# LepistaBioinformatics/blutils

Hardware: NVIDIA B200
Metric: consensus_queries_per_s (higher is better)
Workload: dtype u8

## Files before the change

### blutils_b200/csrc/blu_kernels.cu

```cuda
#include <cuda_runtime.h>

#include <climits>
#include <cstdio>

#include "blu_kernels.h"

namespace blu {

namespace {

constexpr int kRowCap = kWin / 26 + 16;
constexpr int kLongThreads = 512;
constexpr int kLongWarps = kLongThreads / 32;

__device__ __forceinline__ uint32_t smem_u32(const void* p) { return (uint32_t)__cvta_generic_to_shared(p); }
__device__ __forceinline__ uint32_t atoms_add(void* addr, uint32_t v) {
    uint32_t old;
    asm volatile("atom.shared.add.u32 %0, [%1], %2;" : "=r"(old) : "r"(smem_u32(addr)), "r"(v) : "memory");
    return old;
}

__device__ __forceinline__ void mbar_init(unsigned long long* bar, uint32_t count) {
    asm volatile("mbarrier.init.shared::cta.b64 [%0], %1;" ::"r"(smem_u32(bar)), "r"(count) : "memory");
    asm volatile("fence.mbarrier_init.release.cluster;" ::: "memory");
// ... 1377 lines not shown
    bool single;
    if (diverge > 0) {
        identity = __longlong_as_double((long long)S.bcast64[0]), idx = diverge - 1, level = diverge, single = false;
    } else {
        identity = ref.pident, idx = m - 1, level = m - 1, single = true;
    }
    for (int i = tid; i < n2; i += kLongThreads) {
        Q.bord[i] = i < g ? (uint16_t)i : (uint16_t)0xFFFFu;
        if (i < g) Q.key[i] = T.bean_key[T.lin_off[rows[Q.order[i]].lin] + level];
    }
    __syncthreads();
    block_bitonic_u16(Q.bord, n2, [&](int a, int b) { return Q.key[a] != Q.key[b] ? Q.key[a] < Q.key[b] : a < b; });
    for (int i = tid; i < g; i += kLongThreads) {
        const bool head = i == 0 || Q.key[Q.bord[i]] != Q.key[Q.bord[i - 1]];
        const bool kept = head || !acc_equal(rows[Q.order[Q.bord[i]]], rows[Q.order[Q.bord[i - 1]]], p.text);
        Q.tmp[i] = (uint16_t)((head ? 1 : 0) | (kept ? 2 : 0));
    }
    __syncthreads();
    const int nb = block_excl_scan_u16(Q.hb, g, [&](int i) { return (int)(Q.tmp[i] & 1u); }, S.scan_tot);
    const int nkept = block_excl_scan_u16(Q.kp, g, [&](int i) { return (int)((Q.tmp[i] >> 1) & 1u); }, S.scan_tot);
    for (int i = tid; i < g; i += kLongThreads) {
        const bool head = (Q.tmp[i] & 1u) != 0;
        if (head) Q.st[Q.hb[i]] = (uint16_t)i;
    }
    if (tid == 0) Q.st[nb] = (uint16_t)g;
    __syncthreads();
    for (int i = tid; i < g; i += kLongThreads) Q.hb[i] = (uint16_t)(Q.hb[i] + (Q.tmp[i] & 1u));
    int nb2 = 2;
    while (nb2 < nb) nb2 <<= 1;
    for (int j = tid; j < nb2; j += kLongThreads) Q.bsort[j] = j < nb ? (uint16_t)j : (uint16_t)0xFFFFu;
    __syncthreads();
    block_bitonic_u16(Q.bsort, nb2, [&](int a, int b) {
        const int oa = (int)Q.st[a + 1] - (int)Q.st[a], ob = (int)Q.st[b + 1] - (int)Q.st[b];
        if (oa != ob) return oa > ob;
        const uint32_t pa = T.lin_off[rows[Q.order[Q.bord[Q.st[a]]]].lin] + (uint32_t)level, pb = T.lin_off[rows[Q.order[Q.bord[Q.st[b]]]].lin] + (uint32_t)level;
        const uint32_t ia = T.ident_rank[pa], ib = T.ident_rank[pb];
        if (ia != ib) return ia < ib;
        return Q.key[Q.bord[Q.st[a]]] < Q.key[Q.bord[Q.st[b]]];
    });
    block_excl_scan_u16(Q.tmp, nb, [&](int j) { const int bb = Q.bsort[j]; return (int)Q.kp[Q.st[bb + 1]] - (int)Q.kp[Q.st[bb]]; }, S.scan_tot);
    for (int j = tid; j < nb; j += kLongThreads) Q.abeg[Q.bsort[j]] = Q.tmp[j];
    if (tid == 0) {
        const unsigned long long ri = atomicAdd(&p.ctr->rec_count, 1ull);
        const unsigned long long bb = atomicAdd(&p.ctr->bean_used, (unsigned long long)nb);
        const unsigned long long ab = atomicAdd(&p.ctr->acc_used, (unsigned long long)nkept);
        S.bcast64[1] = ri, S.bcast64[2] = bb, S.bcast64[3] = ab;
        if (ri >= p.rec_cap || bb + (unsigned long long)nb > p.bean_cap || ab + (unsigned long long)nkept > p.acc_cap) {
            p.ctr->cap_overflow = 1;
            S.bcast64[1] = ~0ull;
        }
    }
    __syncthreads();
    if (S.bcast64[1] == ~0ull) return DE_NONE;
    const unsigned long long ri = S.bcast64[1], bean_base = S.bcast64[2], acc_base = S.bcast64[3];
    for (int j = tid; j < nb; j += kLongThreads) {
        const int bb = Q.bsort[j];
        blu_bean bn;
        bn.first_lineage = rows[Q.order[Q.bord[Q.st[bb]]]].lin;
        bn.occurrences = (uint32_t)((int)Q.st[bb + 1] - (int)Q.st[bb]);
        bn.acc_begin = Q.abeg[bb];
        bn.n_acc = (uint32_t)((int)Q.kp[Q.st[bb + 1]] - (int)Q.kp[Q.st[bb]]);
        p.beans[bean_base + j] = bn;
    }
    for (int i = tid; i < g; i += kLongThreads)
        if (Q.kp[i + 1] != Q.kp[i]) {
            const int bb = (int)Q.hb[i] - 1;
            const TopRow& x = rows[Q.order[Q.bord[i]]];
            p.accs[acc_base + Q.abeg[bb] + (Q.kp[i] - Q.kp[Q.st[bb]])].ref = (x.acc_off << 16) | (unsigned long long)x.acc_len;
        }
    if (tid == 0) {
        blu_record* rec = p.records + ri;
        rec->query_off = s;
        rec->query_len = qlen;
        rec->n_rows = (uint32_t)nrows;
        rec->bit_score = mx;
        rec->perc_identity = ref.pident;
        rec->ref_lineage = ref.lin;
        rec->bean_base = (uint32_t)bean_base;
        rec->n_beans = (uint32_t)nb;
        rec->acc_base = (uint32_t)acc_base;
        rec->status = 1;
        rec->single_match = 0;
        rec->bean_level = (int8_t)level;
        rec->pad[0] = rec->pad[1] = 0;
        apply_cutoffs(T, ref.lin, identity, single && nb == 1, idx, rec);
    }
    return DE_NONE;
}

__global__ void __launch_bounds__(kLongThreads, 1) longrun_kernel(const __grid_constant__ RunParams p) {
    if (p.ctr->n_defer == 0) return;
    extern __shared__ __align__(128) uint8_t smem_raw[];
    LongSmem& S = *reinterpret_cast<LongSmem*>(smem_raw);
    const int tid = threadIdx.x, warp = tid >> 5, lane = tid & 31;
    const unsigned long long p_begin = p.begin == kBeginFromCounters ? p.ctr->next_begin : p.begin;
    if (tid == 0) mbar_init(&S.mbar, 1);
    __syncthreads();
    uint32_t phase = 0;
    const unsigned n_defer = p.ctr->n_defer < p.defer_cap ? p.ctr->n_defer : p.defer_cap;
    TopRow* const rows = p.big_rows + (size_t)blockIdx.x * kLongTopCap;
    unsigned long long* const cand = p.big_cand + (size_t)blockIdx.x * kLongTopCap;

    while (true) {
        __syncthreads();
        if (tid == 0) S.bcast[0] = (int)atomicAdd(&p.ctr->work_ticket, 1u);
        __syncthreads();
        const unsigned wi = (unsigned)S.bcast[0];
        if (wi >= n_defer) break;
        const unsigned long long entry = p.defer[wi];
        const unsigned long long s = entry >> 1;
        if (entry & 1) {
            if (tid == 0) {
                int head = 1;
                if (s > p_begin) {
                    long long q = (long long)s - 1;
                    while (q >= (long long)p_begin && p.text[q] == '\n') q--;
                    if (q >= (long long)p_begin) {
                        long long st = q;
                        while (st > (long long)p_begin && p.text[st - 1] != '\n') st--;
                        head = 0;
                        for (unsigned long long i = 0;; i++) {
                            if (s + i >= p.end || (unsigned long long)st + i > (unsigned long long)q) {
                                head = 1;
                                break;
                            }
                            uint8_t a = p.text[st + i], b = p.text[s + i];
                            if (a != b) {
                                head = 1;
                                break;
                            }
                            if (a == '\t') break;
                        }
                    }
                }
                S.bcast[1] = head;
            }
            __syncthreads();
            if (!S.bcast[1]) continue;
        }
        if (tid == 0) {
            int qn = 0;
            while (qn < kQidCache && s + qn < p.end) {
                const uint8_t b = p.text[s + qn];
                S.qid[qn++] = b;
                if (b == '\t') break;
            }
            S.bcast[4] = (qn > 0 && S.qid[qn - 1] == '\t') ? qn : 0;
        }
        __syncthreads();
        const int qn = S.bcast[4];
        long long mx = LLONG_MIN;
        long long cnt = 0, nrows = 0;
        unsigned long long cur = s;
        bool ended = false, hit_end = false, fail = false;
        while (true) {
            LongScan sc = long_scan(S, p, s, cur, phase, qn);
            if (sc.giant && sc.d == 0 && sc.ncomplete == 0) {
                if (!sc.at_end || p.final_chunk) {
                    if (tid == 0) report(p.ctr, DE_CARRY_TOO_BIG, cur);
                    fail = true;
                }
                hit_end = true;
                break;
            }
            const unsigned long long lo = cur & ~15ull;
            long long lm = LLONG_MIN;
            for (int i = tid; i < sc.d; i += kLongThreads) {
                const long long b = S.scan.bits[i];
                lm = b > lm ? b : lm;
            }
#pragma unroll
            for (int dd = 16; dd > 0; dd >>= 1) {
                const long long om = __shfl_xor_sync(0xffffffffu, lm, dd);
                lm = om > lm ? om : lm;
            }
            if (lane == 0) S.red_max[warp] = lm;
            __syncthreads();
            long long wm = LLONG_MIN;
            for (int i = 0; i < kLongWarps; i++) wm = S.red_max[i] > wm ? S.red_max[i] : wm;
            if (sc.d > 0 && wm > mx) {
                mx = wm;
                cnt = 0;
            }
            for (int b0 = 0; b0 < sc.d; b0 += kLongThreads) {
                const int i = b0 + tid;
                const bool top = i < sc.d && S.scan.bits[i] == mx;
                const unsigned bal = __ballot_sync(0xffffffffu, top);
                if (lane == 0) S.red_cnt[warp] = __popc(bal);
                __syncthreads();
                long long before = cnt;
                int total = 0;
                for (int k = 0; k < kLongWarps; k++) {
                    if (k < warp) before += S.red_cnt[k];
                    total += S.red_cnt[k];
                }
                if (top) {
                    const long long pos = before + __popc(bal & ((1u << lane) - 1u));
                    if (pos < kLongTopCap)
                        cand[pos] = ((lo + S.scan.W.row_s[i]) << 16) |
                                    (unsigned long long)(uint32_t)((int)S.scan.W.row_e[i + sc.eskip] - (int)S.scan.W.row_s[i]);
                }
                cnt += total;
                __syncthreads();
            }
            nrows += sc.d;
            if (sc.d < sc.ncomplete) {
                ended = true;
                break;
            }
            if (sc.at_end) {
                hit_end = true;
                break;
            }
            cur = sc.next;
        }
        if (fail) continue;
        if (!ended && hit_end && !p.final_chunk) {
            if (tid == 0) atomicMin(&p.ctr->tail_start, s);
            continue;
        }
        if (nrows == 0) continue;
        if (cnt > kLongTopCap) {
            if (tid == 0) report(p.ctr, DE_TOPGROUP_TOO_BIG, s);
            continue;
        }
        const int gcount = (int)cnt;
        uint32_t my_err = 0;
        unsigned long long my_off = 0;
        for (int i = tid; i < gcount; i += kLongThreads) {
            const unsigned long long off = cand[i] >> 16;
            const uint32_t err = heavy_parse_row(p.text + off, (int)(cand[i] & 0xFFFFull), off, p.T, rows[i]);
            if (err && !my_err) my_err = err, my_off = off;
        }
        if (my_err) report_soft(p.ctr, my_err, my_off);
        uint32_t soft = __syncthreads_or(my_err != 0) ? 1u : 0u;
        uint32_t ql = 0;
        if (qn > 0)
            ql = (uint32_t)(qn - 1);
        else
            while (s + ql < p.end && p.text[s + ql] != '\t') ql++;
        if (!soft && gcount > 1) {
            const uint32_t ce = long_consensus(S, p, rows, gcount, s, ql, (unsigned long long)nrows, mx);
            if (ce) {
                if (tid == 0) report_soft(p.ctr, ce, s);
                soft = 1;
            }
        }
        if (tid == 0 && (soft || gcount == 1)) {
            const unsigned long long ri = atomicAdd(&p.ctr->rec_count, 1ull);
            unsigned long long bb = 0, ab = 0;
            if (!soft) {
                bb = atomicAdd(&p.ctr->bean_used, 1ull);
                ab = atomicAdd(&p.ctr->acc_used, 1ull);
            }
            if (ri >= p.rec_cap || bb + 1 > p.bean_cap || ab + 1 > p.acc_cap)
                p.ctr->cap_overflow = 1;
            else {
                blu_record* rec = p.records + ri;
                rec->query_off = s;
                rec->query_len = ql;
                rec->n_rows = (uint32_t)nrows;
                rec->keep_mask = 0;
                rec->perc_identity = 0.0;
                rec->bit_score = mx;
                rec->ref_lineage = 0;
                rec->bean_base = (uint32_t)bb;
                rec->n_beans = 0;
                rec->acc_base = (uint32_t)ab;
                rec->status = 0;
                rec->single_match = rec->mutated = 0;
                rec->reached_pos = 0, rec->allowed_pos = -1, rec->bean_level = 0;
                rec->pad[0] = rec->pad[1] = 0;
                if (!soft) {
                    QueryOut out{rec, p.beans + bb, p.accs + ab};
                    const uint32_t ce = consensus_single(rows[0], p.T, out);
                    if (ce) {
                        report_soft(p.ctr, ce, s);
                        rec->status = 0, rec->n_beans = 0;
                    }
                }
            }
        }
    }
}

__device__ __forceinline__ int cmp_u64(unsigned long long a, unsigned long long b) { return a < b ? -1 : (a > b ? 1 : 0); }

__device__ __forceinline__ int cmp_acc(unsigned long long a0, unsigned long long a1, unsigned alen, unsigned long long aoff, unsigned long long b0,
                                       unsigned long long b1, unsigned blen, unsigned long long boff, const uint8_t* text) {
    int c = cmp_u64(a0, b0);
    if (c) return c;
    c = cmp_u64(a1, b1);
    if (c) return c;
    if (alen > 16 && blen > 16) {
        const unsigned n = alen < blen ? alen : blen;
        for (unsigned i = 16; i < n; i++) {
            int d = (int)text[aoff + i] - (int)text[boff + i];
            if (d) return d;
        }
    }
    return (int)alen - (int)blen;
}

constexpr int kConsThreads = 128;

struct ConsLane {
    unsigned long long keep_mask;
    double perc_identity;
    uint32_t ref_lineage;
    int nb, nkept;
    int reached, allowed, level;
    bool mutated, single, ok;
    bool leader, keeps;
    blu_bean bean;
    int bean_idx, acc_idx;
    unsigned long long acc_ref;
};

template <int W>
__device__ __forceinline__ ConsLane cons_compute(const PostParams& p, bool valid, int g, unsigned long long slot, unsigned long long query_off, int lane) {
    const unsigned FULL = 0xffffffffu;
    const LinTables& T = p.T;
    const int sl = lane & (W - 1);
    const int gsh = lane & ~(W - 1);
    const unsigned WM = W == 32 ? FULL : ((1u << (W & 31)) - 1u);
    auto seg = [&](unsigned b) { return W == 32 ? b : ((b >> gsh) & WM); };
    const unsigned ltm = (1u << sl) - 1u;
    ConsLane o;
    o.keep_mask = 0, o.perc_identity = 0.0, o.ref_lineage = 0, o.nb = 0, o.nkept = 0, o.reached = 0, o.allowed = -1, o.level = 0;
    o.mutated = false, o.single = false, o.ok = false, o.leader = false, o.keeps = false, o.bean_idx = 0, o.acc_idx = 0, o.acc_ref = 0;
    o.bean.first_lineage = 0, o.bean.occurrences = 0, o.bean.acc_begin = 0, o.bean.n_acc = 0;
    const bool on = valid && sl < g;
    TopRow r;
    r.pident = 0.0, r.alnlen = 0, r.acc_off = 0, r.lin = 0, r.acc_len = 0, r.lin_len = 0;
    uint32_t pos0 = 0, jerr = 0;
    if (on) {
        const TopRowRaw raw = p.toprows[slot + sl];
        const unsigned long long off = raw.acc_off;
        if (raw.dec_frac == kTopRowUnparsed)
            jerr = off + (unsigned long long)raw.acc_len <= p.text_end ? heavy_parse_row(p.text + off, (int)raw.acc_len, off, T, r) : (uint32_t)DE_INTERNAL;
        else
            jerr = join_top_row(raw, T, r);
        if (jerr)
            report_soft(p.ctr, jerr, off);
        else
            pos0 = T.lin_off[r.lin];
    }
    bool failed = seg(__ballot_sync(FULL, jerr != 0)) != 0;
    const bool live = valid && !failed;
    unsigned long long k0 = 0, k1 = 0;
    if (on && !failed && g > 1) {
        const unsigned n = r.acc_len;
        const uint32_t* wp = reinterpret_cast<const uint32_t*>(p.text + (r.acc_off & ~3ull));
        const uint32_t sh8 = (uint32_t)(r.acc_off & 3ull) * 8u;
        const uint32_t w0 = wp[0], w1 = wp[1], w2 = wp[2], w3 = wp[3], w4 = wp[4];
        const uint32_t q0 = __byte_perm(__funnelshift_r(w0, w1, sh8), 0u, 0x0123), q1 = __byte_perm(__funnelshift_r(w1, w2, sh8), 0u, 0x0123),
                       q2 = __byte_perm(__funnelshift_r(w2, w3, sh8), 0u, 0x0123), q3 = __byte_perm(__funnelshift_r(w3, w4, sh8), 0u, 0x0123);
        k0 = ((unsigned long long)q0 << 32) | (unsigned long long)q1;
        k1 = ((unsigned long long)q2 << 32) | (unsigned long long)q3;
        if (n < 16) k1 = n > 8 ? (k1 & (~0ull << (8u * (16u - n)))) : 0ull;
        if (n < 8) k0 = n > 0 ? (k0 & (~0ull << (8u * (8u - n)))) : 0ull;
    }
    int gmax = live ? g : 0;
#pragma unroll
    for (int d = 16; d > 0; d >>= 1) {
        const int t = __shfl_xor_sync(FULL, gmax, d);
        gmax = t > gmax ? t : gmax;
    }
    if (gmax > 1) {
        int rank = 0;
        for (int j = 0; j < gmax; j++) {
            const int len_j = __shfl_sync(FULL, (int)r.lin_len, j, W);
            const double pid_j = __shfl_sync(FULL, r.pident, j, W);
            const long long aln_j = __shfl_sync(FULL, (long long)r.alnlen, j, W);
            const unsigned long long k0_j = __shfl_sync(FULL, k0, j, W), k1_j = __shfl_sync(FULL, k1, j, W);
            const unsigned alen_j = __shfl_sync(FULL, (unsigned)r.acc_len, j, W);
            const unsigned long long off_j = __shfl_sync(FULL, (unsigned long long)r.acc_off, j, W);
            if (on && live && j < g && j != sl) {
                bool lt;
                if (len_j != (int)r.lin_len)
                    lt = len_j < (int)r.lin_len;
                else if (pid_j < r.pident)
                    lt = true;
                else if (pid_j > r.pident)
                    lt = false;
                else if (aln_j != (long long)r.alnlen)
                    lt = aln_j < (long long)r.alnlen;
                else {
                    const int c = cmp_acc(k0_j, k1_j, alen_j, off_j, k0, k1, r.acc_len, r.acc_off, p.text);
                    lt = c < 0 || (c == 0 && j < sl);
                }
                if (lt) rank++;
            }
        }
        int src = sl;
        for (int j = 0; j < gmax; j++) {
            const int rj = __shfl_sync(FULL, rank, j, W);
            if (on && live && j < g && rj == sl) src = j;
        }
        r.pident = __shfl_sync(FULL, r.pident, src, W);
        r.alnlen = __shfl_sync(FULL, (long long)r.alnlen, src, W);
        r.acc_off = __shfl_sync(FULL, (unsigned long long)r.acc_off, src, W);
        r.lin = __shfl_sync(FULL, r.lin, src, W);
        r.acc_len = (uint16_t)__shfl_sync(FULL, (unsigned)r.acc_len, src, W);
        r.lin_len = (uint16_t)__shfl_sync(FULL, (unsigned)r.lin_len, src, W);
        pos0 = __shfl_sync(FULL, pos0, src, W);
        k0 = __shfl_sync(FULL, k0, src, W);
        k1 = __shfl_sync(FULL, k1, src, W);
    }
    const int ref_lane = p.strategy == BLU_STRATEGY_CAUTIOUS ? 0 : (g > 0 ? g - 1 : 0);
    const int m = __shfl_sync(FULL, (int)r.lin_len, 0, W);
    const uint32_t lin0 = __shfl_sync(FULL, r.lin, 0, W);
    const unsigned dm = seg(__ballot_sync(FULL, on && r.lin != lin0));
    const bool differ = live && g > 1 && dm != 0;
    int diverge = -1;
    {
        int mmax = differ ? m : 0;
#pragma unroll
        for (int d = 16; d > 0; d >>= 1) {
            const int t = __shfl_xor_sync(FULL, mmax, d);
            mmax = t > mmax ? t : mmax;
        }
        for (int i0 = 0; i0 < mmax; i0 += 4) {
            uint32_t key[4];
#pragma unroll
            for (int u = 0; u < 4; u++) key[u] = (on && differ && diverge < 0 && i0 + u < m) ? T.lvl_key[pos0 + i0 + u] : 0u;
#pragma unroll
            for (int u = 0; u < 4; u++) {
                const uint32_t key0 = __shfl_sync(FULL, key[u], 0, W);
                const bool mism = on && differ && i0 + u < m && key[u] != key0;
                const unsigned bm = seg(__ballot_sync(FULL, mism));
                if (bm && diverge < 0) diverge = i0 + u;
            }
            if (__all_sync(FULL, !differ || diverge >= 0)) break;
        }
    }
    if (live && diverge == 0) {
        if (sl == 0) report_soft(p.ctr, DE_ROOT_DISAGREE, query_off);
        failed = true;
    }
    double identity;
    int idx, level;
    bool single;
    const double ref_pid = __shfl_sync(FULL, r.pident, ref_lane, W);
    double mxp = on ? r.pident : 0.0;
    if (!(mxp > 0.0)) mxp = 0.0;
#pragma unroll
    for (int d = W / 2; d > 0; d >>= 1) {
        const double t = __shfl_xor_sync(FULL, mxp, d);
        mxp = t > mxp ? t : mxp;
    }
    if (diverge > 0)
        identity = mxp, idx = diverge - 1, level = diverge, single = false;
    else
        identity = ref_pid, idx = m - 1, level = m - 1, single = true;
    const bool go = valid && !failed;
    unsigned long long mkey = 0x8000000000000000ull | (unsigned long long)lane;
    uint32_t bkey = 0, irank = 0;
    if (on && go) {
        bkey = T.bean_key[pos0 + level];
        irank = T.ident_rank[pos0 + level];
        mkey = ((unsigned long long)(gsh + 1) << 32) | (unsigned long long)bkey;
    }
    const unsigned grp = seg(__match_any_sync(FULL, mkey));
    const unsigned below = grp & ltm;
    const bool leader = on && go && below == 0;
    const int occ = __popc(grp);
    const int pl = below ? 31 - __clz(below) : sl;
    const unsigned long long pk0 = __shfl_sync(FULL, k0, pl, W), pk1 = __shfl_sync(FULL, k1, pl, W);
    const unsigned plen = __shfl_sync(FULL, (unsigned)r.acc_len, pl, W);
    const unsigned long long poff = __shfl_sync(FULL, (unsigned long long)r.acc_off, pl, W);
    bool dropped = false;
    if (on && go && below) dropped = plen == r.acc_len && cmp_acc(pk0, pk1, plen, poff, k0, k1, r.acc_len, r.acc_off, p.text) == 0;
    const unsigned kept = seg(__ballot_sync(FULL, on && go && !dropped));
    const int nacc_bean = __popc(grp & kept);
    const int my_idx = __popc(grp & kept & ltm);
    const unsigned lm = seg(__ballot_sync(FULL, leader));
    int brank = 0, acc_begin = 0;
    {
        int jmax = go ? g : 0;
#pragma unroll
        for (int d = 16; d > 0; d >>= 1) {
            const int t = __shfl_xor_sync(FULL, jmax, d);
            jmax = t > jmax ? t : jmax;
        }
        for (int j = 0; j < jmax; j++) {
            const int occ_j = __shfl_sync(FULL, occ, j, W);
            const uint32_t ir_j = __shfl_sync(FULL, irank, j, W), bk_j = __shfl_sync(FULL, bkey, j, W);
            const int na_j = __shfl_sync(FULL, nacc_bean, j, W);
            if (leader && ((lm >> j) & 1u) && j != sl) {
                const bool better = occ_j != occ ? occ_j > occ : (ir_j != irank ? ir_j < irank : bk_j < bkey);
                if (better) {
                    brank++;
                    acc_begin += na_j;
                }
            }
        }
    }
    const int my_begin = __shfl_sync(FULL, acc_begin, grp ? __ffs(grp) - 1 : 0, W);
    const int nb = __popc(lm);
    const uint32_t ref_lin = __shfl_sync(FULL, r.lin, ref_lane, W);
    const uint32_t ref_o = __shfl_sync(FULL, pos0, ref_lane, W);
    const int ref_k = __shfl_sync(FULL, (int)r.lin_len, ref_lane, W);
    unsigned long long ge = 0, notgt = 0;
    {
        int kmax = go ? ref_k : 0;
#pragma unroll
        for (int d = 16; d > 0; d >>= 1) {
            const int t = __shfl_xor_sync(FULL, kmax, d);
            kmax = t > kmax ? t : kmax;
        }
        for (int j0 = 0; j0 < kmax; j0 += W) {
            const int j = j0 + sl;
            const bool in = go && j < ref_k;
            double c = 0.0;
            if (in) c = T.cut[ref_o + j];
            const unsigned b_ge = seg(__ballot_sync(FULL, in && identity >= c));
            const unsigned b_ng = seg(__ballot_sync(FULL, in && !(identity > c)));
            ge |= (unsigned long long)b_ge << j0;
            notgt |= (unsigned long long)b_ng << j0;
        }
    }
    if (go && g == 1 && !ge) {
        if (sl == 0) report_soft(p.ctr, DE_EMPTY_ADJUSTED, query_off);
        failed = true;
    }
    o.ok = valid && !failed;
    if (!o.ok) return o;
    o.leader = leader;
    o.keeps = on && !dropped;
    o.bean.first_lineage = r.lin, o.bean.occurrences = (uint32_t)occ, o.bean.acc_begin = (uint32_t)acc_begin, o.bean.n_acc = (uint32_t)nacc_bean;
    o.bean_idx = brank;
    o.acc_idx = my_begin + my_idx;
    o.acc_ref = (r.acc_off << 16) | (unsigned long long)r.acc_len;
    o.nb = nb;
    o.nkept = __popc(kept);
    o.ref_lineage = ref_lin;
    o.level = level;
    if (g == 1) {
        const int last = 63 - __clzll((long long)ge);
        o.keep_mask = ge, o.perc_identity = ref_pid, o.single = true, o.mutated = false, o.reached = last, o.allowed = -1, o.level = last;
    } else {
        const int allowed = notgt ? (__ffsll((long long)notgt) - 1) : -1;
        unsigned long long mask = ge;
        if (!(single && nb == 1)) {
            unsigned long long mk = 0, rest = ge;
            for (int n = 0; n <= idx && rest; n++) {
                const unsigned long long low = rest & (~rest + 1);
                mk |= low;
                rest ^= low;
            }
            mask = mk;
        }
        const int last = mask ? 63 - __clzll((long long)mask) : -1;
        o.keep_mask = mask, o.perc_identity = ref_pid, o.single = false, o.allowed = allowed, o.reached = last >= 0 ? last : idx;
        o.mutated = sl == 0 && allowed >= 0 && T.rank_cls[ref_o + idx] != T.allowed_cls[ref_o + allowed];
    }
    return o;
}

__device__ __forceinline__ void cons_write_record(blu_record* rec, const ConsLane& o) {
    if (o.ok) {
        rec->keep_mask = o.keep_mask;
        rec->perc_identity = o.perc_identity;
        rec->ref_lineage = o.ref_lineage;
        rec->n_beans = (uint32_t)o.nb;
        rec->single_match = o.single ? 1 : 0;
        rec->mutated = o.mutated ? 1 : 0;
        rec->reached_pos = (int8_t)o.reached;
        rec->allowed_pos = (int8_t)o.allowed;
        rec->bean_level = (int8_t)o.level;
        rec->status = 1;
    } else {
        rec->bean_base = 0, rec->n_beans = 0, rec->acc_base = 0;
        rec->status = 0;
    }
}

constexpr int kConsWarps = kConsThreads / 32;
constexpr int kConsBatch = 32;

struct ConsStage {
    blu_bean beans[kConsBatch][8];
    unsigned long long accs[kConsBatch][8];
    int nb[kConsBatch], na[kConsBatch];
    uint8_t list[kConsBatch];
};

#ifndef BLU_CONS_SORTED
#define BLU_CONS_SORTED 1
#endif

#ifndef BLU_CONS_MINB
#define BLU_CONS_MINB 8
#endif
__global__ void __launch_bounds__(kConsThreads, BLU_CONS_MINB) consensus_kernel(const __grid_constant__ PostParams p) {
    __shared__ ConsStage stage_all[kConsWarps];
    const unsigned FULL = 0xffffffffu;
    const int tid = threadIdx.x, lane = tid & 31, warp = tid >> 5;
    const uint32_t lt = (1u << lane) - 1u;
    const int sub = lane >> 3, sl8 = lane & 7;
    ConsStage& St = stage_all[warp];
    if (p.ctr->cap_overflow) return;
    const unsigned long long rb = p.ctr->post_done;
    unsigned long long re = p.ctr->rec_count;
    if (re > p.rec_cap) re = p.rec_cap;
    unsigned long long rows_sum = 0;
    const unsigned long long gw = (unsigned long long)blockIdx.x * kConsWarps + (unsigned long long)warp;
    const unsigned long long wstride = (unsigned long long)gridDim.x * kConsWarps * kConsBatch;
    for (unsigned long long base = rb + gw * kConsBatch; base < re; base += wstride) {
        const unsigned long long qi = base + (unsigned long long)lane;
        blu_record* rec = p.records + qi;
        int g = 0, cls = 0;
        unsigned long long slot = 0, qoff = 0;
        if (qi < re) {
            rows_sum += rec->n_rows;
            if (rec->status == 2) {
                g = (int)rec->n_beans;
                slot = rec->bean_base;
                qoff = rec->query_off;
                if (g >= 1 && slot + (unsigned long long)g <= p.slot_cap) cls = g <= 8 ? 1 : (g <= 32 ? 2 : 3);
            }
        }
        St.nb[lane] = 0, St.na[lane] = 0;
        if (cls == 3) {
            report(p.ctr, DE_INTERNAL, qoff);
            rec->status = 0, rec->n_beans = 0;
        }
        int n8 = 0;
        {
            int pos = 0;
#pragma unroll
            for (int k = 1; k <= 8; k++) {
                const unsigned mk = __ballot_sync(FULL, cls == 1 && (BLU_CONS_SORTED ? g == k : k == 1));
                if (BLU_CONS_SORTED ? k < g : false) pos += __popc(mk);
                if (BLU_CONS_SORTED ? k == g : k == 1) pos += __popc(mk & lt);
                n8 += __popc(mk);
            }
            if (cls == 1) St.list[pos] = (uint8_t)lane;
        }
        unsigned m32 = __ballot_sync(FULL, cls == 2);
        __syncwarp();
        for (int t = 0; t * 4 < n8; t++) {
            const int at = t * 4 + sub;
            const bool valid = at < n8;
            const int q = valid ? (int)St.list[at] : 0;
            const int gq = __shfl_sync(FULL, g, q);
            const unsigned long long slotq = __shfl_sync(FULL, slot, q), qoffq = __shfl_sync(FULL, qoff, q);
            const ConsLane o = cons_compute<8>(p, valid, gq, slotq, qoffq, lane);
            if (o.ok && o.leader) St.beans[q][o.bean_idx] = o.bean;
            if (o.ok && o.keeps) St.accs[q][o.acc_idx] = o.acc_ref;
            if (valid && sl8 == 0) {
                St.nb[q] = o.ok ? o.nb : 0;
                St.na[q] = o.ok ? o.nkept : 0;
                cons_write_record(p.records + base + (unsigned long long)q, o);
            }
        }
        __syncwarp();
        const int vb = St.nb[lane], va = St.na[lane];
        int ib = vb, ia = va;
#pragma unroll
        for (int d = 1; d < 32; d <<= 1) {
            const int tb = __shfl_up_sync(FULL, ib, d), ta = __shfl_up_sync(FULL, ia, d);
            if (lane >= d) ib += tb, ia += ta;
        }
        const int tot_b = __shfl_sync(FULL, ib, 31), tot_a = __shfl_sync(FULL, ia, 31);
        unsigned long long bb = 0, ab = 0;
        if (lane == 0) {
            if (tot_b) bb = atomicAdd(&p.ctr->bean_used, (unsigned long long)tot_b);
            if (tot_a) ab = atomicAdd(&p.ctr->acc_used, (unsigned long long)tot_a);
        }
        bb = __shfl_sync(FULL, bb, 0), ab = __shfl_sync(FULL, ab, 0);
        const bool fits = bb + (unsigned long long)tot_b <= p.bean_cap && ab + (unsigned long long)tot_a <= p.acc_cap;
        if (!fits && lane == 0) p.ctr->cap_overflow = 1;
        const unsigned long long my_b = bb + (unsigned long long)(ib - vb), my_a = ab + (unsigned long long)(ia - va);
        if (fits) {
            if (vb > 0) {
                rec->bean_base = (uint32_t)my_b;
                rec->acc_base = (uint32_t)my_a;
            }
            for (int t = 0; t < kConsBatch / 4; t++) {
                const int qslot = t * 4 + sub;
                const unsigned long long qb = __shfl_sync(FULL, my_b, qslot), qa = __shfl_sync(FULL, my_a, qslot);
                const int nbq = __shfl_sync(FULL, vb, qslot), naq = __shfl_sync(FULL, va, qslot);
                if (sl8 < nbq) p.beans[qb + sl8] = St.beans[qslot][sl8];
                if (sl8 < naq) p.accs[qa + sl8].ref = St.accs[qslot][sl8];
            }
        }
        __syncwarp();
        while (m32) {
            const int q = __ffs(m32) - 1;
            m32 &= m32 - 1;
            const int gw2 = __shfl_sync(FULL, g, q);
            const unsigned long long slotw = __shfl_sync(FULL, slot, q), qoffw = __shfl_sync(FULL, qoff, q);
            blu_record* recw = p.records + base + (unsigned long long)q;
            const ConsLane ow = cons_compute<32>(p, true, gw2, slotw, qoffw, lane);
            unsigned long long wb = 0, wa = 0;
            int wfits = 1;
            if (lane == 0 && ow.ok) {
                wb = atomicAdd(&p.ctr->bean_used, (unsigned long long)ow.nb);
                wa = atomicAdd(&p.ctr->acc_used, (unsigned long long)ow.nkept);
                wfits = wb + (unsigned long long)ow.nb <= p.bean_cap && wa + (unsigned long long)ow.nkept <= p.acc_cap;
                if (!wfits) p.ctr->cap_overflow = 1;
            }
            wb = __shfl_sync(FULL, wb, 0), wa = __shfl_sync(FULL, wa, 0), wfits = __shfl_sync(FULL, wfits, 0);
            if (ow.ok && wfits) {
                if (ow.leader) p.beans[wb + ow.bean_idx] = ow.bean;
                if (ow.keeps) p.accs[wa + ow.acc_idx].ref = ow.acc_ref;
            }
            if (lane == 0) {
                cons_write_record(recw, ow);
                if (ow.ok && wfits) recw->bean_base = (uint32_t)wb, recw->acc_base = (uint32_t)wa;
            }
        }
    }
#pragma unroll
    for (int d = 16; d > 0; d >>= 1) rows_sum += __shfl_xor_sync(FULL, rows_sum, d);
    if (lane == 0 && rows_sum) atomicAdd(&p.ctr->n_rows, rows_sum);
}

__global__ void __launch_bounds__(256) gather_kernel(const __grid_constant__ PostParams p) {
    const unsigned FULL = 0xffffffffu;
    const int lane = threadIdx.x & 31;
    if (p.ctr->cap_overflow) return;
    const unsigned long long rb = p.ctr->post_done;
    unsigned long long re = p.ctr->rec_count;
    if (re > p.rec_cap) re = p.rec_cap;
    const unsigned long long wstride = (unsigned long long)gridDim.x * (blockDim.x >> 5) * 32ull;
    for (unsigned long long base = rb + ((unsigned long long)blockIdx.x * (blockDim.x >> 5) + (threadIdx.x >> 5)) * 32ull; base < re; base += wstride) {
        const unsigned long long i = base + lane;
        const bool live = i < re;
        blu_record* rec = p.records + i;
        unsigned long long bytes = 0, qoff = 0, abase = 0;
        uint32_t qlen = 0, nacc = 0;
        if (live) {
            qoff = rec->query_off, qlen = rec->query_len;
            bytes = qlen;
            if (rec->status == 1) {
                abase = rec->acc_base;
                const uint32_t nbn = rec->n_beans;
                if (nbn) {
                    const blu_bean lb = p.beans[(unsigned long long)rec->bean_base + nbn - 1];
                    nacc = lb.acc_begin + lb.n_acc;
                }
                for (uint32_t a = 0; a < nacc; a++) bytes += (uint32_t)(p.accs[abase + a].ref & 0xFFFFull);
            }
        }
        unsigned long long inc = bytes;
#pragma unroll
        for (int d = 1; d < 32; d <<= 1) {
            const unsigned long long t = __shfl_up_sync(FULL, inc, d);
            if (lane >= d) inc += t;
        }
        const unsigned long long total = __shfl_sync(FULL, inc, 31);
        unsigned long long wbase = 0;
        if (lane == 31 && total) wbase = atomicAdd(&p.ctr->pool_used, total);
        wbase = __shfl_sync(FULL, wbase, 31);
        if (!p.pool) continue;
        if (wbase + total > p.pool_cap) {
            if (lane == 0) p.ctr->cap_overflow = 1;
            continue;
        }
        const unsigned long long mine = wbase + inc - bytes;
        uint32_t namax = nacc;
#pragma unroll
        for (int d = 16; d > 0; d >>= 1) {
            const uint32_t t = __shfl_xor_sync(FULL, namax, d);
            namax = t > namax ? t : namax;
        }
        unsigned long long cur = mine;
        for (int rr = 0; rr < 32; rr++) {
            const unsigned long long so = __shfl_sync(FULL, qoff, rr), dst = __shfl_sync(FULL, cur, rr);
            const uint32_t n = __shfl_sync(FULL, qlen, rr);
            for (uint32_t k = lane; k < n; k += 32) p.pool[dst + k] = p.text[so + k];
        }
        if (live) rec->query_off = mine;
        cur += qlen;
        for (uint32_t a = 0; a < namax; a++) {
            unsigned long long ref = 0;
            if (a < nacc) ref = p.accs[abase + a].ref;
            for (int rr = 0; rr < 32; rr++) {
                const unsigned long long rf = __shfl_sync(FULL, ref, rr), dst = __shfl_sync(FULL, cur, rr);
                const uint32_t n = (uint32_t)(rf & 0xFFFFull);
                const unsigned long long so = rf >> 16;
                for (uint32_t k = lane; k < n; k += 32) p.pool[dst + k] = p.text[so + k];
            }
            if (a < nacc) {
                p.accs[abase + a].ref = (cur << 16) | (ref & 0xFFFFull);
                cur += (uint32_t)(ref & 0xFFFFull);
            }
        }
    }
}

__global__ void __launch_bounds__(256) dup_kernel(const __grid_constant__ DupParams p) {
    if (p.ctr->cap_overflow) return;
    const unsigned long long rb = p.ctr->post_done;
    unsigned long long n = p.ctr->rec_count;
    if (n > p.rec_cap) n = p.rec_cap;
    for (unsigned long long i = rb + (unsigned long long)blockIdx.x * blockDim.x + threadIdx.x; i < n; i += (unsigned long long)gridDim.x * blockDim.x) {
        blu_record& r = p.records[i];
        if (r.query_off + (unsigned long long)r.query_len > p.strings_len) continue;
        if (p.table) {
            unsigned long long h = 0xcbf29ce484222325ull;
            const uint8_t* q = p.strings + r.query_off;
            for (unsigned k = 0; k < r.query_len; k++) {
                h ^= q[k];
                h *= 0x100000001b3ull;
            }
            h = mix64(h ^ r.query_len);
            if (h == 0) h = 1;
            if (p.hashes) p.hashes[i] = h;
            unsigned slot = (unsigned)h & p.mask;
            for (unsigned t = 0; t <= p.mask; t++) {
                const unsigned long long old = atomicCAS(p.table + slot, 0ull, h);
                if (old == 0ull) break;
                if (old == h) {
                    p.ctr->dup_found = 1;
                    break;
                }
                slot = (slot + 1) & p.mask;
            }
        }
        if (p.ref_delta) {
            r.query_off = (unsigned long long)((long long)r.query_off + p.ref_delta);
            if (r.status == 1 && r.n_beans) {
                const blu_bean lb = p.beans[(unsigned long long)r.bean_base + r.n_beans - 1];
                const unsigned nacc = lb.acc_begin + lb.n_acc;
                for (unsigned a = 0; a < nacc; a++) {
                    blu_acc& ac = p.accs[(unsigned long long)r.acc_base + a];
                    ac.ref = (unsigned long long)((long long)ac.ref + p.ref_delta * 65536);
                }
            }
        }
    }
}

__global__ void __launch_bounds__(256) dup_merge_kernel(const unsigned long long* hashes, unsigned long long n, unsigned long long* table, uint32_t mask,
                                                        unsigned int* dup_found) {
    for (unsigned long long i = (unsigned long long)blockIdx.x * blockDim.x + threadIdx.x; i < n; i += (unsigned long long)gridDim.x * blockDim.x) {
        const unsigned long long h = hashes[i];
        unsigned slot = (unsigned)h & mask;
        for (unsigned t = 0; t <= mask; t++) {
            const unsigned long long old = atomicCAS(table + slot, 0ull, h);
            if (old == 0ull) break;
            if (old == h) {
                *dup_found = 1;
                break;
            }
            slot = (slot + 1) & mask;
        }
    }
}

__global__ void __launch_bounds__(256) fanout_kernel(const __grid_constant__ FanoutParams p) {
    const Counters* s = p.src;
    const unsigned long long rb = s->post_done;
    unsigned long long re = s->rec_count;
    if (re > p.rec_cap) re = p.rec_cap;
    if (!s->cap_overflow && re > rb) {
        constexpr unsigned long long kPer = sizeof(blu_record) / sizeof(uint4);
        const unsigned long long n = (re - rb) * kPer;
        const uint4* src = reinterpret_cast<const uint4*>(p.src_records + rb);
        const unsigned long long stride = (unsigned long long)gridDim.x * blockDim.x;
        for (unsigned long long i = (unsigned long long)blockIdx.x * blockDim.x + threadIdx.x; i < n * (unsigned long long)p.n_dst; i += stride) {
            const unsigned long long d = i / n, j = i - d * n;
            reinterpret_cast<uint4*>(p.dst_records[d] + rb)[j] = src[j];
        }
    }
    if (blockIdx.x == 0 && (int)threadIdx.x < p.n_dst) {
        Counters* d = p.dst[threadIdx.x];
        if (d->post_done != rb) report(d, DE_INTERNAL, 0);
        d->rec_count = s->rec_count;
        d->slot_count = s->slot_count;
        d->n_defer = s->n_defer;
        if (s->tail_start < d->tail_start) d->tail_start = s->tail_start;
        if (s->err_code && !d->err_code) d->err_code = s->err_code, d->err_off = s->err_off;
        if (s->cap_overflow) d->cap_overflow = 1;
    }
}

__global__ void advance_kernel(const AdvanceParams p) {
    Counters* c = p.ctr;
    unsigned long long n = c->rec_count;
    if (n > p.rec_cap) n = p.rec_cap;
    c->post_done = n;
    c->next_begin = c->tail_start != ~0ull ? c->tail_start : p.range_end;
    if (p.snapshot) {
        *p.snapshot = *c;
        __threadfence_system();
    }
    c->n_defer = 0;
    c->work_ticket = 0;
    c->tail_start = ~0ull;
}

}

cudaError_t kernels_set_attributes() {
    cudaError_t e = cudaFuncSetAttribute(tile_kernel, cudaFuncAttributeMaxDynamicSharedMemorySize, (int)sizeof(StreamSmem));
    if (e != cudaSuccess) return e;
    return cudaFuncSetAttribute(longrun_kernel, cudaFuncAttributeMaxDynamicSharedMemorySize, (int)sizeof(LongSmem));
}

int tile_kernel_grid(int device) {
    int sms = 148;
    cudaDeviceGetAttribute(&sms, cudaDevAttrMultiProcessorCount, device);
    return kTileCtasPerSm * sms;
}

cudaError_t launch_tile_kernel(const RunParams& p, int grid, cudaStream_t s) {
    tile_kernel<<<grid, kTileThreads, sizeof(StreamSmem), s>>>(p);
    return cudaGetLastError();
}

cudaError_t launch_longrun_kernel(const RunParams& p, int grid, cudaStream_t s) {
    longrun_kernel<<<grid, kLongThreads, sizeof(LongSmem), s>>>(p);
    return cudaGetLastError();
}

cudaError_t launch_consensus_kernel(const PostParams& p, int sms, cudaStream_t s) {
    consensus_kernel<<<sms * 16, kConsThreads, 0, s>>>(p);
    return cudaGetLastError();
}

cudaError_t launch_gather_kernel(const PostParams& p, int sms, cudaStream_t s) {
    gather_kernel<<<sms * 8, 256, 0, s>>>(p);
    return cudaGetLastError();
}

cudaError_t launch_dup_kernel(const DupParams& p, int sms, cudaStream_t s) {
    dup_kernel<<<sms * 8, 256, 0, s>>>(p);
    return cudaGetLastError();
}

cudaError_t launch_fanout_kernel(const FanoutParams& p, int sms, cudaStream_t s) {
    fanout_kernel<<<sms * 4, 256, 0, s>>>(p);
    return cudaGetLastError();
}

cudaError_t launch_dup_merge_kernel(const unsigned long long* hashes, unsigned long long n, unsigned long long* table, uint32_t mask,
                                    unsigned int* dup_found, int sms, cudaStream_t s) {
    if (!n) return cudaSuccess;
    dup_merge_kernel<<<sms * 8, 256, 0, s>>>(hashes, n, table, mask, dup_found);
    return cudaGetLastError();
}

cudaError_t launch_advance_kernel(const AdvanceParams& p, cudaStream_t s) {
    advance_kernel<<<1, 1, 0, s>>>(p);
    return cudaGetLastError();
}

}
```

### blutils_b200/csrc/blu_kernels.h

```cpp
#pragma once
#include <cuda_runtime.h>
#include <stdint.h>

#include "blu_core.cuh"

namespace blu {

struct Counters {
    unsigned long long rec_count;
    unsigned long long slot_count;
    unsigned long long bean_used;
    unsigned long long acc_used;
    unsigned long long pool_used;
    unsigned long long post_done;
    unsigned long long next_begin;
    unsigned long long err_off;
    unsigned long long soft_off;
    unsigned long long tail_start;
    unsigned long long n_rows;
    unsigned int n_defer;
    unsigned int work_ticket;
    unsigned int err_code;
    unsigned int soft_code;
    unsigned int dup_found;
    unsigned int cap_overflow;
    unsigned int pad0;
    unsigned int pad;
};

constexpr uint64_t kBeginFromCounters = ~0ull;

struct RunParams {
    const uint8_t* text;
    uint64_t begin, end;
    int final_chunk;
    int strategy;
    LinTables T;
    blu_record* records;
    uint64_t rec_cap;
    TopRowRaw* toprows;
    uint64_t slot_cap;
    blu_bean* beans;
    uint64_t bean_cap;
    blu_acc* accs;
    uint64_t acc_cap;
    uint64_t* defer;
    uint32_t defer_cap;
    TopRow* big_rows;
    unsigned long long* big_cand;
    Counters* ctr;
};

struct PostParams {
    blu_record* records;
    uint64_t rec_cap;
    const TopRowRaw* toprows;
    uint64_t slot_cap;
    blu_bean* beans;
    uint64_t bean_cap;
    blu_acc* accs;
    uint64_t acc_cap;
    const uint8_t* text;
    uint64_t text_end;
    uint8_t* pool;
    uint64_t pool_cap;
    LinTables T;
    int strategy;
    Counters* ctr;
};

struct DupParams {
    blu_record* records;
    uint64_t rec_cap;
    const blu_bean* beans;
    blu_acc* accs;
    const uint8_t* strings;
    uint64_t strings_len;
    unsigned long long* table;
    uint32_t mask;
    unsigned long long* hashes;
    long long ref_delta;
    Counters* ctr;
};

constexpr int kMaxConfigs = 8;

struct FanoutParams {
    const Counters* src;
    const blu_record* src_records;
    Counters* dst[kMaxConfigs - 1];
    blu_record* dst_records[kMaxConfigs - 1];
    int n_dst;
    uint64_t rec_cap;
};

struct AdvanceParams {
    Counters* ctr;
    uint64_t rec_cap;
    uint64_t range_end;
    Counters* snapshot;
};

#ifndef BLU_TILE_BYTES
#define BLU_TILE_BYTES 32768
#endif
#ifndef BLU_TILE_CTAS
#define BLU_TILE_CTAS 2
#endif
#ifndef BLU_TILE_THREADS
#define BLU_TILE_THREADS 512
#endif
constexpr int kTile = BLU_TILE_BYTES;
constexpr int kBack = 1024;
constexpr int kTileThreads = BLU_TILE_THREADS;
constexpr int kTileCtasPerSm = BLU_TILE_CTAS;
constexpr int kWin = 60416;

int tile_kernel_grid(int device);
cudaError_t launch_tile_kernel(const RunParams& p, int grid, cudaStream_t s);
cudaError_t launch_longrun_kernel(const RunParams& p, int grid, cudaStream_t s);
cudaError_t launch_consensus_kernel(const PostParams& p, int sms, cudaStream_t s);
cudaError_t launch_gather_kernel(const PostParams& p, int sms, cudaStream_t s);
cudaError_t launch_dup_kernel(const DupParams& p, int sms, cudaStream_t s);
cudaError_t launch_fanout_kernel(const FanoutParams& p, int sms, cudaStream_t s);
cudaError_t launch_advance_kernel(const AdvanceParams& p, cudaStream_t s);
cudaError_t launch_dup_merge_kernel(const unsigned long long* hashes, unsigned long long n, unsigned long long* table, uint32_t mask,
                                    unsigned int* dup_found, int sms, cudaStream_t s);
constexpr int kLongTopCap = 8192;
cudaError_t kernels_set_attributes();

int regroup_device(const uint8_t* d_text, uint64_t n, cudaStream_t s, uint8_t** d_out, uint64_t* out_n, uint64_t* n_rows_out);

}
```

Measured before the change: 258.6 million.

## Prejoin consensus rows warp-wide, use dynamic batch tickets, widen dup hashing

The consensus kernel now parses and joins every top row of a batch cooperatively across all 32 lanes up front, storing lineage, position and accession keys in a repacked shared stage that is reused for bean and accession staging. Work distribution moves from a static grid stride to an atomic ticket per batch, and the grid is sized from occupancy. The dup kernel hash changes from byte-wise FNV to a word-at-a-time hash. These aim to raise lane utilisation in the 8-wide path and balance load, at the cost of an atomic per batch and a different hash function.

```diff
diff --git a/blutils_b200/csrc/blu_kernels.cu b/blutils_b200/csrc/blu_kernels.cu
--- a/blutils_b200/csrc/blu_kernels.cu
+++ b/blutils_b200/csrc/blu_kernels.cu
@@ -1703,7 +1703,36 @@
     return (int)alen - (int)blen;
 }
 
+__device__ __forceinline__ void acc_key(const uint8_t* text, unsigned long long off, unsigned n, unsigned long long& k0, unsigned long long& k1) {
+    const uint32_t* wp = reinterpret_cast<const uint32_t*>(text + (off & ~3ull));
+    const uint32_t sh8 = (uint32_t)(off & 3ull) * 8u;
+    const uint32_t w0 = wp[0], w1 = wp[1], w2 = wp[2], w3 = wp[3], w4 = wp[4];
+    const uint32_t q0 = __byte_perm(__funnelshift_r(w0, w1, sh8), 0u, 0x0123), q1 = __byte_perm(__funnelshift_r(w1, w2, sh8), 0u, 0x0123),
+                   q2 = __byte_perm(__funnelshift_r(w2, w3, sh8), 0u, 0x0123), q3 = __byte_perm(__funnelshift_r(w3, w4, sh8), 0u, 0x0123);
+    k0 = ((unsigned long long)q0 << 32) | (unsigned long long)q1;
+    k1 = ((unsigned long long)q2 << 32) | (unsigned long long)q3;
+    if (n < 16) k1 = n > 8 ? (k1 & (~0ull << (8u * (16u - n)))) : 0ull;
+    if (n < 8) k0 = n > 0 ? (k0 & (~0ull << (8u * (8u - n)))) : 0ull;
+}
+
+__device__ __noinline__ uint32_t heavy_parse_top_row(const uint8_t* text, unsigned long long off, unsigned len, const LinTables& T, TopRow& r) {
+    return heavy_parse_row(text + off, (int)len, off, T, r);
+}
+
 constexpr int kConsThreads = 128;
+constexpr int kConsWarps = kConsThreads / 32;
+constexpr int kConsBatch = 32;
+constexpr int kConsRows = kConsBatch * 8;
+constexpr uint32_t kJoinFailed = 0xFFFFFFFFu;
+
+struct ConsStage {
+    unsigned long long w0[kConsRows], w1[kConsRows];
+    uint32_t lin[kConsRows], pos[kConsRows];
+    uint16_t llen[kConsRows];
+    uint8_t nb[kConsBatch], na[kConsBatch];
+    uint8_t ro[kConsBatch];
+    uint8_t list[kConsBatch];
+};
 
 struct ConsLane {
     unsigned long long keep_mask;
@@ -1719,7 +1748,8 @@
 };
 
 template <int W>
-__device__ __forceinline__ ConsLane cons_compute(const PostParams& p, bool valid, int g, unsigned long long slot, unsigned long long query_off, int lane) {
+__device__ __forceinline__ ConsLane cons_compute(const PostParams& p, const ConsStage& St, int ro, bool valid, int g, unsigned long long slot,
+                                                 unsigned long long query_off, int lane) {
     const unsigned FULL = 0xffffffffu;
     const LinTables& T = p.T;
     const int sl = lane & (W - 1);
@@ -1735,33 +1765,38 @@
     TopRow r;
     r.pident = 0.0, r.alnlen = 0, r.acc_off = 0, r.lin = 0, r.acc_len = 0, r.lin_len = 0;
     uint32_t pos0 = 0, jerr = 0;
+    unsigned long long k0 = 0, k1 = 0;
     if (on) {
         const TopRowRaw raw = p.toprows[slot + sl];
         const unsigned long long off = raw.acc_off;
-        if (raw.dec_frac == kTopRowUnparsed)
-            jerr = off + (unsigned long long)raw.acc_len <= p.text_end ? heavy_parse_row(p.text + off, (int)raw.acc_len, off, T, r) : (uint32_t)DE_INTERNAL;
-        else
-            jerr = join_top_row(raw, T, r);
-        if (jerr)
-            report_soft(p.ctr, jerr, off);
-        else
-            pos0 = T.lin_off[r.lin];
+        if constexpr (W == 8) {
+            const int row = ro + sl;
+            const uint32_t lin = St.lin[row];
+            if (lin == kJoinFailed) {
+                jerr = St.llen[row];
+            } else {
+                if (raw.dec_frac == kTopRowUnparsed)
+                    heavy_parse_top_row(p.text, off, raw.acc_len, T, r);
+                else
+                    r.pident = toprow_pident(raw), r.alnlen = raw.alnlen, r.acc_off = off, r.acc_len = (uint16_t)raw.acc_len;
+                r.lin = lin, r.lin_len = St.llen[row];
+                pos0 = St.pos[row];
+                if (g > 1) k0 = St.w0[row], k1 = St.w1[row];
+            }
+        } else {
+            if (raw.dec_frac == kTopRowUnparsed)
+                jerr = off + (unsigned long long)raw.acc_len <= p.text_end ? heavy_parse_top_row(p.text, off, raw.acc_len, T, r) : (uint32_t)DE_INTERNAL;
+            else
+                jerr = join_top_row(raw, T, r);
+            if (!jerr) {
+                pos0 = T.lin_off[r.lin];
+                acc_key(p.text, r.acc_off, r.acc_len, k0, k1);
+            }
+        }
+        if (jerr) report_soft(p.ctr, jerr, off);
     }
     bool failed = seg(__ballot_sync(FULL, jerr != 0)) != 0;
     const bool live = valid && !failed;
-    unsigned long long k0 = 0, k1 = 0;
-    if (on && !failed && g > 1) {
-        const unsigned n = r.acc_len;
-        const uint32_t* wp = reinterpret_cast<const uint32_t*>(p.text + (r.acc_off & ~3ull));
-        const uint32_t sh8 = (uint32_t)(r.acc_off & 3ull) * 8u;
-        const uint32_t w0 = wp[0], w1 = wp[1], w2 = wp[2], w3 = wp[3], w4 = wp[4];
-        const uint32_t q0 = __byte_perm(__funnelshift_r(w0, w1, sh8), 0u, 0x0123), q1 = __byte_perm(__funnelshift_r(w1, w2, sh8), 0u, 0x0123),
-                       q2 = __byte_perm(__funnelshift_r(w2, w3, sh8), 0u, 0x0123), q3 = __byte_perm(__funnelshift_r(w3, w4, sh8), 0u, 0x0123);
-        k0 = ((unsigned long long)q0 << 32) | (unsigned long long)q1;
-        k1 = ((unsigned long long)q2 << 32) | (unsigned long long)q3;
-        if (n < 16) k1 = n > 8 ? (k1 & (~0ull << (8u * (16u - n)))) : 0ull;
-        if (n < 8) k0 = n > 0 ? (k0 & (~0ull << (8u * (8u - n)))) : 0ull;
-    }
     int gmax = live ? g : 0;
 #pragma unroll
     for (int d = 16; d > 0; d >>= 1) {
@@ -1978,16 +2013,6 @@
     }
 }
 
-constexpr int kConsWarps = kConsThreads / 32;
-constexpr int kConsBatch = 32;
-
-struct ConsStage {
-    blu_bean beans[kConsBatch][8];
-    unsigned long long accs[kConsBatch][8];
-    int nb[kConsBatch], na[kConsBatch];
-    uint8_t list[kConsBatch];
-};
-
 #ifndef BLU_CONS_SORTED
 #define BLU_CONS_SORTED 1
 #endif
@@ -2007,9 +2032,11 @@
     unsigned long long re = p.ctr->rec_count;
     if (re > p.rec_cap) re = p.rec_cap;
     unsigned long long rows_sum = 0;
-    const unsigned long long gw = (unsigned long long)blockIdx.x * kConsWarps + (unsigned long long)warp;
-    const unsigned long long wstride = (unsigned long long)gridDim.x * kConsWarps * kConsBatch;
-    for (unsigned long long base = rb + gw * kConsBatch; base < re; base += wstride) {
+    unsigned batch = 0;
+    if (lane == 0) batch = atomicAdd(&p.ctr->cons_ticket, 1u);
+    batch = __shfl_sync(FULL, batch, 0);
+    for (unsigned long long base = rb + (unsigned long long)batch * kConsBatch; base < re; base = rb + (unsigned long long)batch * kConsBatch) {
+        if (lane == 0) batch = atomicAdd(&p.ctr->cons_ticket, 1u);
         const unsigned long long qi = base + (unsigned long long)lane;
         blu_record* rec = p.records + qi;
         int g = 0, cls = 0;
@@ -2042,18 +2069,64 @@
         }
         unsigned m32 = __ballot_sync(FULL, cls == 2);
         __syncwarp();
+        const int eq = lane < n8 ? (int)St.list[lane] : 0;
+        const int gq0 = __shfl_sync(FULL, g, eq);
+        const int eg = lane < n8 ? gq0 : 0;
+        const unsigned long long eslot = __shfl_sync(FULL, slot, eq);
+        int ero = eg;
+#pragma unroll
+        for (int d = 1; d < 32; d <<= 1) {
+            const int t = __shfl_up_sync(FULL, ero, d);
+            if (lane >= d) ero += t;
+        }
+        const int nrows = __shfl_sync(FULL, ero, 31);
+        ero -= eg;
+        if (lane < n8) St.ro[eq] = (uint8_t)ero;
+        for (int c0 = 0; c0 < nrows; c0 += 32) {
+            const unsigned starts = __reduce_or_sync(FULL, lane < n8 && ero >= c0 && ero < c0 + 32 ? 1u << (ero - c0) : 0u);
+            const int before = __popc(__ballot_sync(FULL, lane < n8 && ero < c0));
+            const int e = before + __popc(starts & (FULL >> (31 - lane))) - 1;
+            const int row = c0 + lane;
+            const int ro_e = __shfl_sync(FULL, ero, e & 31), g_e = __shfl_sync(FULL, eg, e & 31);
+            const unsigned long long slot_e = __shfl_sync(FULL, eslot, e & 31);
+            if (row < nrows) {
+                const TopRowRaw raw = p.toprows[slot_e + (unsigned long long)(row - ro_e)];
+                const unsigned long long off = raw.acc_off;
+                TopRow r;
+                uint32_t jerr;
+                if (raw.dec_frac == kTopRowUnparsed)
+                    jerr = off + (unsigned long long)raw.acc_len <= p.text_end ? heavy_parse_top_row(p.text, off, raw.acc_len, p.T, r) : (uint32_t)DE_INTERNAL;
+                else
+                    jerr = join_top_row(raw, p.T, r);
+                if (jerr) {
+                    St.lin[row] = kJoinFailed, St.llen[row] = (uint16_t)jerr;
+                } else {
+                    St.lin[row] = r.lin, St.llen[row] = r.lin_len, St.pos[row] = p.T.lin_off[r.lin];
+                    if (g_e > 1) {
+                        unsigned long long k0, k1;
+                        acc_key(p.text, r.acc_off, r.acc_len, k0, k1);
+                        St.w0[row] = k0, St.w1[row] = k1;
+                    }
+                }
+            }
+        }
+        __syncwarp();
         for (int t = 0; t * 4 < n8; t++) {
             const int at = t * 4 + sub;
             const bool valid = at < n8;
             const int q = valid ? (int)St.list[at] : 0;
             const int gq = __shfl_sync(FULL, g, q);
             const unsigned long long slotq = __shfl_sync(FULL, slot, q), qoffq = __shfl_sync(FULL, qoff, q);
-            const ConsLane o = cons_compute<8>(p, valid, gq, slotq, qoffq, lane);
-            if (o.ok && o.leader) St.beans[q][o.bean_idx] = o.bean;
-            if (o.ok && o.keeps) St.accs[q][o.acc_idx] = o.acc_ref;
+            const int roq = __shfl_sync(FULL, ero, at & 31);
+            const ConsLane o = cons_compute<8>(p, St, roq, valid, gq, slotq, qoffq, lane);
+            if (o.ok && o.leader) {
+                St.w0[roq + o.bean_idx] = (unsigned long long)o.bean.first_lineage | ((unsigned long long)o.bean.occurrences << 32);
+                St.w1[roq + o.bean_idx] = (unsigned long long)o.bean.acc_begin | ((unsigned long long)o.bean.n_acc << 32);
+            }
+            if (o.ok && o.keeps) St.lin[roq + o.acc_idx] = (uint32_t)o.acc_ref, St.pos[roq + o.acc_idx] = (uint32_t)(o.acc_ref >> 32);
             if (valid && sl8 == 0) {
-                St.nb[q] = o.ok ? o.nb : 0;
-                St.na[q] = o.ok ? o.nkept : 0;
+                St.nb[q] = (uint8_t)(o.ok ? o.nb : 0);
+                St.na[q] = (uint8_t)(o.ok ? o.nkept : 0);
                 cons_write_record(p.records + base + (unsigned long long)q, o);
             }
         }
@@ -2084,8 +2157,12 @@
                 const int qslot = t * 4 + sub;
                 const unsigned long long qb = __shfl_sync(FULL, my_b, qslot), qa = __shfl_sync(FULL, my_a, qslot);
                 const int nbq = __shfl_sync(FULL, vb, qslot), naq = __shfl_sync(FULL, va, qslot);
-                if (sl8 < nbq) p.beans[qb + sl8] = St.beans[qslot][sl8];
-                if (sl8 < naq) p.accs[qa + sl8].ref = St.accs[qslot][sl8];
+                const int row = (int)St.ro[qslot] + sl8;
+                if (sl8 < nbq) {
+                    const unsigned long long b0 = St.w0[row], b1 = St.w1[row];
+                    p.beans[qb + sl8] = blu_bean{(uint32_t)b0, (uint32_t)(b0 >> 32), (uint32_t)b1, (uint32_t)(b1 >> 32)};
+                }
+                if (sl8 < naq) p.accs[qa + sl8].ref = (unsigned long long)St.lin[row] | ((unsigned long long)St.pos[row] << 32);
             }
         }
         __syncwarp();
@@ -2095,7 +2172,7 @@
             const int gw2 = __shfl_sync(FULL, g, q);
             const unsigned long long slotw = __shfl_sync(FULL, slot, q), qoffw = __shfl_sync(FULL, qoff, q);
             blu_record* recw = p.records + base + (unsigned long long)q;
-            const ConsLane ow = cons_compute<32>(p, true, gw2, slotw, qoffw, lane);
+            const ConsLane ow = cons_compute<32>(p, St, 0, true, gw2, slotw, qoffw, lane);
             unsigned long long wb = 0, wa = 0;
             int wfits = 1;
             if (lane == 0 && ow.ok) {
@@ -2114,6 +2191,7 @@
                 if (ow.ok && wfits) recw->bean_base = (uint32_t)wb, recw->acc_base = (uint32_t)wa;
             }
         }
+        batch = __shfl_sync(FULL, batch, 0);
     }
 #pragma unroll
     for (int d = 16; d > 0; d >>= 1) rows_sum += __shfl_xor_sync(FULL, rows_sum, d);
@@ -2194,6 +2272,27 @@
     }
 }
 
+__device__ __forceinline__ unsigned long long id_hash(const uint8_t* q, unsigned n) {
+    unsigned long long h = 0xcbf29ce484222325ull;
+    if (n) {
+        const uintptr_t a = reinterpret_cast<uintptr_t>(q);
+        const unsigned long long* wp = reinterpret_cast<const unsigned long long*>(a & ~(uintptr_t)7);
+        const unsigned sh = (unsigned)(a & 7u) * 8u;
+        const unsigned nw = (unsigned)(((a + n - 1) >> 3) - (a >> 3)) + 1u;
+        unsigned long long lo = wp[0];
+        for (unsigned i = 0; 8u * i < n; i++) {
+            const unsigned long long hi = i + 1 < nw ? wp[i + 1] : 0ull;
+            unsigned long long c = sh ? (lo >> sh) | (hi << (64u - sh)) : lo;
+            const unsigned left = n - 8u * i;
+            if (left < 8) c &= (1ull << (8u * left)) - 1ull;
+            h = (h ^ c) * 0x9E3779B97F4A7C15ull;
+            h ^= h >> 29;
+            lo = hi;
+        }
+    }
+    return mix64(h ^ n);
+}
+
 __global__ void __launch_bounds__(256) dup_kernel(const __grid_constant__ DupParams p) {
     if (p.ctr->cap_overflow) return;
     const unsigned long long rb = p.ctr->post_done;
@@ -2203,13 +2302,7 @@
         blu_record& r = p.records[i];
         if (r.query_off + (unsigned long long)r.query_len > p.strings_len) continue;
         if (p.table) {
-            unsigned long long h = 0xcbf29ce484222325ull;
-            const uint8_t* q = p.strings + r.query_off;
-            for (unsigned k = 0; k < r.query_len; k++) {
-                h ^= q[k];
-                h *= 0x100000001b3ull;
-            }
-            h = mix64(h ^ r.query_len);
+            unsigned long long h = id_hash(p.strings + r.query_off, r.query_len);
             if (h == 0) h = 1;
             if (p.hashes) p.hashes[i] = h;
             unsigned slot = (unsigned)h & p.mask;
@@ -2293,6 +2386,7 @@
     }
     c->n_defer = 0;
     c->work_ticket = 0;
+    c->cons_ticket = 0;
     c->tail_start = ~0ull;
 }
 
@@ -2321,7 +2415,11 @@
 }
 
 cudaError_t launch_consensus_kernel(const PostParams& p, int sms, cudaStream_t s) {
-    consensus_kernel<<<sms * 16, kConsThreads, 0, s>>>(p);
+    static const int per_sm = [] {
+        int n = 0;
+        return cudaOccupancyMaxActiveBlocksPerMultiprocessor(&n, consensus_kernel, kConsThreads, 0) == cudaSuccess && n > 0 ? n : 1;
+    }();
+    consensus_kernel<<<sms * per_sm, kConsThreads, 0, s>>>(p);
     return cudaGetLastError();
 }
 
diff --git a/blutils_b200/csrc/blu_kernels.h b/blutils_b200/csrc/blu_kernels.h
--- a/blutils_b200/csrc/blu_kernels.h
+++ b/blutils_b200/csrc/blu_kernels.h
@@ -24,7 +24,7 @@
     unsigned int soft_code;
     unsigned int dup_found;
     unsigned int cap_overflow;
-    unsigned int pad0;
+    unsigned int cons_ticket;
     unsigned int pad;
 };
 
```

Measured after the change: 255.2 million, median of 6. -1.3%, worse.
